# QuanjianSong/UniVST

Measured on AMD Instinct MI355X. Metric: stylized frames/sec, SD-v1.5 16x512x512 @50 DDIM steps, higher is better.
Workload: dtype f16; 1 GPU; sd15_unet_three_branch_pnp_transfer_16x512x512_50ddim; frames=16, branches=3, schedule_steps=53 (wrapping modulo 50), masks=moving disc, blended on steps 0..45, parallelism=single, weights=random-init SD-v1.5 architecture (859M + 201M temporal params), fp16

## Files before the change

### include/univst.h

```cpp
#ifndef UNIVST_H
#define UNIVST_H
#include <stdint.h>
#ifdef __cplusplus
extern "C" {
#endif

#define UNIVST_OK 0
#define UNIVST_ERR_ARG (-1)
#define UNIVST_ERR_HIP (-2)
#define UNIVST_ERR_UNSUPPORTED (-3)
#define UNIVST_ERR_STATE (-4)

#define UNIVST_F16 0
#define UNIVST_F32 1

const char* univst_last_error(void);
#define UNIVST_ABI_VERSION 3
int univst_abi_version(void);

typedef struct univst_unet univst_unet;

typedef struct {
    int in_channels, out_channels;
    int block_out_channels[4];
// ... 146 lines not shown
int univst_motion_load_tensor(univst_motion* h, const char* key, const void* dev_ptr, int dtype, const int64_t* shape, int ndim, void* stream);
int univst_motion_finalize(univst_motion* h, void* stream);
int univst_motion_forward(univst_motion* h, const void* X, void* Y, int B, int F, int N, void* stream);
int univst_motion_query(univst_motion* h, const char* name, double* out);
int univst_temporal_attention(const void* qkv, int64_t ldx, const void* pe_qkv, int B, int F, int N, int heads, int head_dim, void* out, int64_t ldo,
                              void* stream);

int univst_linear(const void* X, int64_t ldx, const void* W, const void* bias, const void* residual, int64_t ldr,
                  void* Y, int64_t ldy, int M, int N, int K, int geglu, void* stream);
int univst_geglu_xres_permute(const void* in, void* out, int rows, int cols, void* stream);
int univst_linear_gated(const void* X, int64_t ldx, const void* W, const void* bias, const void* residual, int64_t ldr, void* Y, int64_t ldy,
                        int M, int N, int K, int act, const void* gate, int64_t ld_gate, int rows_per_gate, void* stream);
int univst_linear_ln(const void* X, int64_t ldx, const void* W, const void* bias, const void* residual, int64_t ldr,
                     void* Y, int64_t ldy, int M, int N, int K, int geglu, const float* ln_stats, float ln_eps,
                     const float* ln_wsum, const float* ln_bias, float* stats_out, void* stream);
int64_t univst_attn2_fused_workspace_bytes(int B, int heads, int head_dim);
int univst_attn2_fused(const void* X, int64_t ldx, const float* ln_stats, float ln_eps, const float* ln_wsum, const float* ln_bias,
                       const void* Wq_frag, int q_prescaled, const void* kv, int B, int T, int64_t rows_per_branch, const void* Wo_frag,
                       const void* bias_o, const void* residual, int64_t ldr, void* Y, int64_t ldy, int64_t M, int C, int heads,
                       float* stats_out, void* workspace, void* stream);
int univst_attn12_fused(const void* attn_out, int64_t ldx, const void* Wp_frag, const void* bias_p, const void* residual_in, int64_t ldr_in, float ln_eps,
                        const float* ln_wsum, const float* ln_bias, const void* Wq_frag, int q_prescaled, const void* kv, int B, int T,
                        int64_t rows_per_branch, const void* Wo_frag, const void* bias_o, void* Y, int64_t ldy, int64_t M, int C, int heads,
                        float* stats_out, void* workspace, void* stream);
int univst_frag_pack(const void* W, void* out, int N, int K, void* stream);
int univst_conv_nhwc(const void* X1, const void* X2, int C1, int C2, int imgs, int Hs, int Ws, int upsample, int stride,
                     int taps, const void* W, const void* bias, const void* rowbias, int rows_per_rowbias,
                     const void* residual, void* Y, int Cout, void* stream);
int univst_conv_nhwc_tapinner(const void* X1, const void* X2, int C1, int C2, int imgs, int Hs, int Ws, int upsample, int stride,
                              const void* W, const void* bias, const void* rowbias, int rows_per_rowbias,
// ... 89 lines not shown
#define UNIVST_PLAN_LN_STATS 8
#define UNIVST_PLAN_STATS_OUT 16
#define UNIVST_PLAN_ACT 32
#define UNIVST_PLAN_GATE 64
#define UNIVST_PLAN_W32_ONLY 128
#define UNIVST_PLAN_W32 256
#define UNIVST_PLAN_GN_OUT 512
#define UNIVST_PLAN_TAPINNER 1024
#define UNIVST_PLAN_Y_UNALIGNED 2048
#define UNIVST_PLAN_WORKSPACE 4096
#define UNIVST_PLAN_GEOM_3X3 0
#define UNIVST_PLAN_GEOM_PAD_END 1
#define UNIVST_PLAN_GEOM_FRAME 2
int univst_debug_gemm_plan(int ncu, int mode, int M, int N, int K, int geglu, int flags, int rows_per_set, int C1, int C2, int Hs, int Ws, int upsample,
                           int stride, int taps, int geom, char* buf, int n);
#define UNIVST_PLAN_SRC_LOGW 1
#define UNIVST_PLAN_EXTRA_KEYS 2
int univst_debug_attention_plan(int BF, int heads, int Nq, int Nkv, int nsrc, int d, int q_prescaled, int flags, int phase, char* buf, int n);

#define UNIVST_GN_PLAN_INTS 16
int univst_debug_groupnorm_plan(int C1, int C2, int64_t rows, int rows_per_stat, int G, int has_fold, int world, int has_producer_stats, int* out_ints);

#ifdef __cplusplus
}
#endif
#endif
```

### univst_amd/_native.py

```python
import ctypes as C
import os
from typing import Optional

import torch

_LIB_PATH = os.environ.get("UNIVST_LIB") or os.path.join(os.path.dirname(os.path.abspath(__file__)), "lib", "libunivst_hip.so")
_lib = None


class UnetCfg(C.Structure):
    _fields_ = [("in_channels", C.c_int), ("out_channels", C.c_int), ("block_out_channels", C.c_int * 4),
                ("layers_per_block", C.c_int), ("cross_attention_dim", C.c_int), ("attention_heads", C.c_int * 4),
                ("norm_num_groups", C.c_int), ("norm_eps", C.c_float), ("flip_sin_to_cos", C.c_int),
                ("freq_shift", C.c_float)]


class ClipCfg(C.Structure):
    _fields_ = [("vocab_size", C.c_int), ("hidden_size", C.c_int), ("intermediate_size", C.c_int), ("num_layers", C.c_int), ("num_heads", C.c_int),
                ("max_positions", C.c_int), ("hidden_act", C.c_int), ("layer_norm_eps", C.c_float), ("projection_dim", C.c_int), ("eos_token_id", C.c_int)]


class T5Cfg(C.Structure):
    _fields_ = [("vocab_size", C.c_int), ("d_model", C.c_int), ("d_ff", C.c_int), ("num_layers", C.c_int), ("num_heads", C.c_int), ("d_kv", C.c_int),
                ("num_buckets", C.c_int), ("max_distance", C.c_int), ("layer_norm_eps", C.c_float)]
# ... 49 lines not shown
    "univst_unet_set_option": (_I, [_P, C.c_char_p, _I]),
    "univst_unet_query": (_I, [_P, C.c_char_p, C.POINTER(C.c_double)]),
    "univst_comm_create": (_I, [_I, _I, _L, C.POINTER(_P)]),
    "univst_comm_handle_bytes": (_I, []),
    "univst_comm_export": (_I, [_P, _P]),
    "univst_comm_connect": (_I, [_P, _P]),
    "univst_comm_connect_local": (_I, [_P, C.POINTER(_P)]),
    "univst_comm_connect_emulated": (_I, [_P, C.c_double, C.c_double]),
    "univst_comm_query": (_I, [_P, C.c_char_p, C.POINTER(C.c_double)]),
    "univst_comm_destroy": (_I, [_P]),
    "univst_comm_allreduce_f32": (_I, [_P, _P, _I, _P]),
    "univst_comm_status": (_I, [_P]),
    "univst_unet_set_comm_native": (_I, [_P, _P]),
    "univst_linear": (_I, [_P, _L, _P, _P, _P, _L, _P, _L, _I, _I, _I, _I, _P]),
    "univst_linear_ln": (_I, [_P, _L, _P, _P, _P, _L, _P, _L, _I, _I, _I, _I, _P, _F, _P, _P, _P, _P]),
    "univst_geglu_xres_permute": (_I, [_P, _P, _I, _I, _P]),
    "univst_frag_pack": (_I, [_P, _P, _I, _I, _P]),
    "univst_vae_create": (_I, [_P, C.POINTER(_P)]),
    "univst_vae_destroy": (_I, [_P]),
    "univst_vae_load_tensor": (_I, [_P, C.c_char_p, _P, _I, C.POINTER(C.c_int64), _I, _P]),
    "univst_vae_finalize": (_I, [_P, _P]),
    "univst_vae_decode": (_I, [_P, _P, _L, _I, _I, _I, _P, _P]),
    "univst_vae_encode": (_I, [_P, _P, _L, _I, _I, _P, _P]),
    "univst_klvae_create": (_I, [_P, C.POINTER(_P)]),
    "univst_klvae_destroy": (_I, [_P]),
    "univst_klvae_load_tensor": (_I, [_P, C.c_char_p, _P, _I, C.POINTER(C.c_int64), _I, _P]),
    "univst_klvae_finalize": (_I, [_P, _P]),
    "univst_klvae_decode": (_I, [_P, _P, _L, _I, _I, _P, _P]),
    "univst_klvae_encode": (_I, [_P, _P, _L, _I, _I, _P, _P]),
    "univst_klvae_query": (_I, [_P, C.c_char_p, C.POINTER(C.c_double)]),
# ... 60 lines not shown
    "univst_latent_adain_apply": (_I, [_P, _P, _P, _L, _P, _I, _I, _I, _P]),
    "univst_axpby": (_I, [_P, _P, _P, _F, _F, _L, _P]),
    "univst_mask_blend": (_I, [_P, _P, _P, _P, _I, _L, _P]),
    "univst_mask_resize": (_I, [_P, _P, _I, _I, _I, _I, _I, _P]),
    "univst_maskprop_workspace_bytes": (_L, [_I, _I, _I]),
    "univst_maskprop_frame": (_I, [_P, _P, _P, _P, _I, _I, _I, _I, _F, _I, _P, _P]),
    "univst_maskprop_finalize": (_I, [_P, _P, _I, _I, _I, _I, _I, _P, _P]),
    "univst_warp_accumulate": (_I, [_P, _P, _P, _P, _P, _I, _I, _F, _P]),
    "univst_warp_window_key": (_I, [_P, _P, _I, _I, _I, _I, _I, _I, _F, _P]),
    "univst_latent_window_smooth": (_I, [_P, _P, _I, _I, _I, _I, _I, _F, _P]),
    "univst_accumulate_u8": (_I, [_P, _P, _L, _P]),
    "univst_window_store": (_I, [_P, _F, _P, _L, _P]),
    "univst_debug_tr16": (_I, [_P, _P]),
    "univst_debug_delay_us": (_I, [C.c_double, _P]),
    "univst_debug_gemm_plan": (_I, [_I] * 16 + [C.c_char_p, _I]),
    "univst_debug_attention_plan": (_I, [_I] * 9 + [C.c_char_p, _I]),
    "univst_debug_groupnorm_plan": (_I, [_I, _I, _L, _I, _I, _I, _I, _I, _P]),
    "univst_profile_enable": (_I, [_I]),
    "univst_profile_symbols": (_I, [_I, C.c_char_p, _I]),
    "univst_profile_collect": (_I, [C.POINTER(C.c_double), C.POINTER(_L), C.POINTER(C.c_double), C.POINTER(C.c_double), _I]),
    "univst_profile_collect_aux": (_I, [C.POINTER(C.c_double), _I]),
}


ABI_VERSION = 3


def lib_path() -> str:
    return _LIB_PATH


def load():
    global _lib
    if _lib is None:
        if not os.path.exists(_LIB_PATH):
            raise RuntimeError(f"{_LIB_PATH} not found: build it with `python __graft_entry__.py build` (or `make`); "
                               "univst_amd has no CPU or eager-PyTorch fallback")
        lib = C.CDLL(_LIB_PATH)
        for name, (res, args) in SIGNATURES.items():
            fn = getattr(lib, name)
            fn.restype = res
            fn.argtypes = args
        if lib.univst_abi_version() != ABI_VERSION:
            raise RuntimeError(f"{_LIB_PATH} has ABI version {lib.univst_abi_version()}, this binding was written against {ABI_VERSION} "
                               "(include/univst.h UNIVST_ABI_VERSION): rebuild the library (`make`)")
        _lib = lib
    return _lib


def check(rc: int, what: str = ""):
    if rc != 0:
        msg = load().univst_last_error().decode(errors="replace")
        raise RuntimeError(f"libunivst_hip {what} failed (code {rc}): {msg}")


# ... 102 lines not shown


def linear_ln(x, w, bias=None, residual=None, geglu=False, out=None, ln=None, stats_out=None, eps=1e-5):
    _f16(x), _f16(w)
    M, K = x.shape
    N = w.shape[0]
    No = N // 2 if geglu else N
    if out is None:
        out = torch.empty(M, No, device=x.device, dtype=torch.float16)
    st, ws, lb = ln if ln is not None else (None, None, None)
    for t in (st, ws, lb, stats_out):
        assert t is None or (t.dtype == torch.float32 and t.is_contiguous())
    check(load().univst_linear_ln(ptr(x), K, ptr(w), ptr(bias), ptr(residual), No, ptr(out), No, M, N, K, int(geglu), ptr(st), eps,
                                  ptr(ws), ptr(lb), ptr(stats_out), stream_ptr()), "linear_ln")
    return out


def conv_nhwc(x1, w, bias=None, x2=None, upsample=False, stride=1, rowbias=None, rows_per_rowbias=1, residual=None):
    _f16(x1), _f16(w)
    imgs, Hs, Ws, C1 = x1.shape
    C2 = 0 if x2 is None else x2.shape[-1]
    Cout, taps, _ = w.shape
    He, We = (Hs * 2, Ws * 2) if upsample else (Hs, Ws)
    Ho = (He - 1) // stride + 1 if taps == 9 else He
    Wo = (We - 1) // stride + 1 if taps == 9 else We
    out = torch.empty(imgs, Ho, Wo, Cout, device=x1.device, dtype=torch.float16)
    check(load().univst_conv_nhwc(ptr(x1), ptr(x2), C1, C2, imgs, Hs, Ws, int(upsample), stride, taps, ptr(w), ptr(bias),
                                  ptr(rowbias), rows_per_rowbias, ptr(residual), ptr(out), Cout, stream_ptr()), "conv_nhwc")
    return out

# ... 315 lines not shown
```

### univst_amd/csrc/abi.hip

```cpp
#include <math.h>
#include <stdarg.h>
#include <stdlib.h>
#include <string.h>

#include <new>

#include "../../include/univst.h"
#include "comm.h"
#include "kernels.h"
#include "unet.h"
#include "vae.h"
#include "raft.h"
#include "clip.h"
#include "t5.h"
#include "motion.h"

static thread_local char g_err[1024] = "";
void uv_set_error(const char* fmt, ...) {
    va_list ap;
    va_start(ap, fmt);
    vsnprintf(g_err, sizeof(g_err), fmt, ap);
    va_end(ap);
}
const char* uv_get_error() { return g_err; }
// ... 42 lines not shown
}
int univst_unet_set_option(univst_unet* h, const char* name, int value) {
    UV_REQUIRE(h && name, "unet_set_option: null argument");
    if (!strcmp(name, "ln_fold")) {
        UV_REQUIRE(value >= 0 && value <= 2, "unet_set_option: ln_fold is 0, 1 or 2");
        h->impl.ln_fold = value;
        return UV_OK;
    }
    if (!strcmp(name, "gn_fold")) {
        h->impl.gn_fold = value != 0;
        return UV_OK;
    }
    if (!strcmp(name, "attn2_fused")) {
        UV_REQUIRE(value >= 0 && value <= 2, "unet_set_option: attn2_fused is 0, 1 or 2");
        h->impl.attn2_fused = value;
        return UV_OK;
    }
    if (!strcmp(name, "gn_producer")) {
        h->impl.gn_producer = value != 0;
        return UV_OK;
    }
    if (!strcmp(name, "chain_bands")) {
        UV_REQUIRE(value >= 0 && value <= 64, "unet_set_option: chain_bands is 0 (auto), 1 (off) or a band count <= 64");
        h->impl.chain_bands = value;
        return UV_OK;
    }
    if (!strcmp(name, "kv_overlap")) {
        h->impl.kv_overlap = value != 0;
        return UV_OK;
    }
// ... 440 lines not shown
    return uv_launch_attn2_fused(p, C, S(s));
}
int univst_linear_ln(const void* X, int64_t ldx, const void* W, const void* bias, const void* R, int64_t ldr, void* Y, int64_t ldy,
                     int M, int N, int K, int geglu, const float* ln_stats, float ln_eps, const float* ln_wsum, const float* ln_bias,
                     float* stats_out, void* s) {
    UV_REQUIRE(X && W && Y, "linear_ln: null argument");
    UV_REQUIRE(!ln_stats || (ln_wsum && ln_bias && K % 160 == 0 && !bias), "linear_ln: a folded LayerNorm needs wsum, lnb (which holds the bias) and K %% 160 == 0");
    UV_REQUIRE((!stats_out || uv_linear_fold_producer_ok(M, N, K)) && (!ln_stats || geglu == 2 || uv_linear_fold_consumer_ok(M, N, K, geglu != 0)),
               "linear_ln: M=%d N=%d K=%d is not taken by the direct 256x320 path (N %% 320 == 0 and >= 150 tiles) nor by the 128-wide path without split-K", M, N, K);
    GemmParams g;
    g.X = H(X); g.ldx = ldx; g.W = H(W); g.bias = H(bias); g.R = H(R); g.ldr = ldr; g.Y = HM(Y); g.ldy = ldy;
    g.M = M; g.N = N; g.K = K; g.geglu = geglu;
    g.ln_stats = ln_stats; g.ln_slots = K / 160; g.ln_eps = ln_eps; g.ln_wsum = ln_wsum; g.ln_bias = ln_bias; g.stats_out = stats_out;
    return uv_launch_gemm(g, 0, S(s));
}
int univst_conv_nhwc(const void* X1, const void* X2, int C1, int C2, int imgs, int Hs, int Ws, int up, int stride, int taps,
                     const void* W, const void* bias, const void* rowbias, int rows_per_rb, const void* R, void* Y, int Cout,
                     void* s) {
    UV_REQUIRE(X1 && W && Y, "conv: null argument");
    UV_REQUIRE((X2 != nullptr) == (C2 > 0), "conv: X2/C2 mismatch");
    UV_REQUIRE(stride == 1 || stride == 2, "conv: stride %d", stride);
    GemmParams g;
    g.X = H(X1); g.X2 = H(X2); g.C1 = C1; g.C2 = C2; g.Hs = Hs; g.Ws = Ws; g.up = up ? 1 : 0; g.stride = stride; g.taps = taps;
    const int He = Hs << g.up, We = Ws << g.up;
    g.Ho = taps == 9 ? (He - 1) / stride + 1 : He;
    g.Wo = taps == 9 ? (We - 1) / stride + 1 : We;
    g.M = imgs * g.Ho * g.Wo; g.N = Cout; g.K = taps * (C1 + C2);
    g.W = H(W); g.bias = H(bias); g.rowbias = H(rowbias); g.rows_per_rb = rows_per_rb > 0 ? rows_per_rb : 1;
    g.R = H(R); g.ldr = Cout; g.Y = HM(Y); g.ldy = Cout;
    return uv_launch_gemm(g, 1, S(s));
// ... 149 lines not shown
        g.korder = on(UNIVST_PLAN_TAPINNER) ? 1 : 0;
    }
    g.ldy = No; g.ldr = No;
    if (on(UNIVST_PLAN_BIAS)) g.bias = h;
    if (on(UNIVST_PLAN_RESIDUAL)) g.R = h;
    if (on(UNIVST_PLAN_ROWBIAS)) g.rowbias = h;
    if (on(UNIVST_PLAN_LN_STATS)) { g.ln_stats = arena; g.ln_wsum = arena; g.ln_bias = arena; g.ln_slots = g.K / 160; }
    if (on(UNIVST_PLAN_STATS_OUT)) g.stats_out = arena;
    if (on(UNIVST_PLAN_ACT)) g.act = 1;
    if (on(UNIVST_PLAN_GATE)) { g.gate = h; g.ld_gate = N; }
    if (on(UNIVST_PLAN_GN_OUT)) { g.gn_out = arena; g.gn_gw = 10; g.gn_G = N / 10; }
    if (on(UNIVST_PLAN_WORKSPACE)) { g.partial = arena; g.partial_bytes = UV_SPLITK_WS_BYTES; }
    if (rows_per_set > 0) { g.w_rows_per_set = rows_per_set; g.bias32 = arena; }
    return uv_gemm_plan_text(g, mode, ncu, buf, n);
}
int univst_debug_attention_plan(int BF, int heads, int Nq, int Nkv, int nsrc, int d, int q_prescaled, int flags, int phase, char* buf, int n) {
    UV_REQUIRE(buf && n > 0 && phase >= 0 && phase <= 2, "debug_attention_plan: null buffer or phase outside 0..2");
    if (Nq == 0 && Nkv == 0) {
        snprintf(buf, (size_t)n, "%s", uv_attention_plan_symbols().c_str());
        return UV_OK;
    }
    alignas(16) static float arena[8];
    half_t* const h = (half_t*)arena;
    AttnParams a;
    a.q = a.k = a.v = h; a.o = h; a.ldq = a.ldkv = a.ldo = (long)heads * d; a.src_idx = (const int*)arena;
    a.nsrc = nsrc; a.BF = BF; a.Nq = Nq; a.Nkv = Nkv; a.heads = heads; a.d = d; a.q_prescaled = q_prescaled != 0;
    if (flags & UNIVST_PLAN_SRC_LOGW) a.src_logw = arena;
    if (flags & UNIVST_PLAN_EXTRA_KEYS) { a.kx = a.vx = h; a.x_idx = (const int*)arena; a.ldkv_x = a.ldkv; a.Nkv_x = 77; }
    if (phase == 1) a.state_out = arena;
    if (phase == 2) a.state_in = arena;
// ... 72 lines not shown
```

### univst_amd/csrc/kernels.h

```cpp
#pragma once
#include "common.h"
#include <string>

struct GemmParams {
    const half_t* X = nullptr;
    const half_t* X2 = nullptr;
    const half_t* W = nullptr;
    const half_t* W32 = nullptr;
    half_t* Y = nullptr;
    long ldx = 0, ldy = 0;
    int M = 0, N = 0, K = 0;
    int C1 = 0, C2 = 0, Hs = 1, Ws = 1, up = 0, Ho = 1, Wo = 1, stride = 1, taps = 1;
    int tapw = 0, pady = 0, padx = 0;
    int korder = 0;
    const half_t* bias = nullptr;
    const half_t* rowbias = nullptr;
    int rows_per_rb = 1;
    long ldrb = 0;
    const half_t* R = nullptr;
    long ldr = 0;
    const half_t* bias2 = nullptr;
    int geglu = 0;
    int act = 0;
    const half_t* gate = nullptr;
// ... 93 lines not shown
struct AttnPlan : UvLaunchPlan {};
GemmPlan uv_gemm_plan(const GemmParams& p, int mode, int ncu);
AttnPlan uv_attention_plan(const AttnParams& p);
int uv_gemm_plan_text(const GemmParams& p, int mode, int ncu, char* buf, int n);
int uv_attention_plan_text(const AttnParams& p, char* buf, int n);
std::string uv_gemm_plan_symbols();
std::string uv_attention_plan_symbols();

int uv_num_cus();
int uv_launch_gemm(const GemmParams& p, int mode, hipStream_t stream);
bool uv_linear_takes_big_direct(long M, int N, int K, long ldx = 0);
bool uv_linear_fold_producer_ok(long M, int N, int K);
bool uv_linear_fold_consumer_ok(long M, int N, int K, bool geglu);
bool uv_geglu_xres_ok(int N, int K, long M = 0);
int uv_launch_geglu_xres_permute(const half_t* in, half_t* out, int rows, int cols, hipStream_t stream);
constexpr size_t UV_SPLITK_WS_BYTES = 128u << 20;
int uv_launch_linear_small(const half_t* x, const half_t* W, const half_t* b, half_t* y, int M, int N, int K, int silu_in,
                           hipStream_t stream);
struct UvGnComm {
    int world = 1;
    float* red = nullptr;
    long byte_off = 0;
    int (*allreduce)(void* user, int64_t byte_off, int count_f32) = nullptr;
    void* user = nullptr;
};
int uv_groupnorm_workspace_floats(int S, int G);
struct UvGnFold {
    const half_t* W = nullptr;
    const half_t* bias = nullptr;
    int N = 0;
// ... 77 lines not shown
```

### univst_amd/csrc/unet.h

```cpp
#pragma once
#include <string>
#include <unordered_map>

#include "../../include/univst.h"
#include "model.h"

struct UNet : WeightStore {
    univst_unet_cfg cfg;
    std::unordered_map<long, int*> idx_tables;
    std::unordered_map<std::string, long> temb_off;
    long temb_total = 0;
    Arena arena;
    bool finalized = false;
    int gn_producer = 1;
    int chain_bands = 1;
    int gn_fold = 1;
    int attn2_fused = 2;
    int ln_fold = 2;
    unsigned* d_counter = nullptr;
    std::unordered_map<std::string, int> temporal_conv_active;
    std::unordered_map<std::string, int> temporal_attn_active;
    int rank = 0, world = 1;
    univst_allreduce_fn allreduce = nullptr;
    univst_kv_exchange_fn kv_exchange = nullptr;
    void* comm_user = nullptr;
    char* comm_ws = nullptr;
    long comm_ws_bytes = 0;
    struct univst_comm* native_comm = nullptr;
    int kv_overlap = 1;
    int emu_wire_gbps = 0, emu_wire_lat_us = 3;
    double emu_wire_us = 0.0;
    hipStream_t xstream = nullptr;
// ... 14 lines not shown
```

### univst_amd/csrc/unet.hip

```cpp
#include <math.h>
#include <string.h>

#include <map>
#include <string>
#include <unordered_map>
#include <vector>

#include "comm.h"
#include "kernels.h"
#include "unet.h"

namespace {

__global__ void permute_conv_weight_t32_kernel(const half_t* __restrict__ in, half_t* __restrict__ out, int Co, int Ci) {
    long i = (long)blockIdx.x * blockDim.x + threadIdx.x;
    long total = (long)Co * Ci * 9;
    if (i >= total) return;
    int j = (int)(i % 32);
    int t = (int)((i / 32) % 9);
    int q = (int)((i / (32 * 9)) % (Ci / 32));
    int o = (int)(i / ((long)Ci * 9));
    out[i] = in[((long)o * Ci + q * 32 + j) * 9 + t];
}
__global__ void geglu_interleave_kernel(const half_t* __restrict__ in, half_t* __restrict__ out, int rows, int cols) {
// ... 618 lines not shown
        g.R = R;
        g.ldr = ldr;
        g.bias2 = bias2;
        g.geglu = geglu;
        if (!g.W || (!bkey.empty() && !ln_in && !wsets && !g.bias)) return u.missing_error("unet");
        g.partial = sk_ws;
        g.partial_bytes = UV_SPLITK_WS_BYTES;
        UV_RUN(uv_launch_gemm(g, 0, s));
        if (g.gn_out) {
            if (emitted) *gst_out = g.gn_out;
            else gst_give_back(M, N);
        }
        return UV_OK;
    }

    struct KvSlots {
        long o_send = 0, o_first = 0, o_prev = 0, o_rfirst = 0, nbytes = 0;
        bool emu = false;
    } kvs;
    int kv_post(const half_t* h, int C, int N) {
        kvs = KvSlots();
        kvs.nbytes = (long)B * N * C * sizeof(half_t);
        const int nslot = u.native_comm ? 6 : 4;
        const long slot = ((u.comm_ws_bytes - 65536) / nslot) & ~255L;
        UV_REQUIRE(kvs.nbytes <= slot, "kv_exchange: comm workspace too small (%ld B per slot, need %ld)", slot, kvs.nbytes);
        const long par = u.native_comm ? uv_comm_kv_parity(u.native_comm) : 0;
        kvs.o_send = 65536;
        kvs.o_first = kvs.o_send + slot;
        kvs.o_prev = kvs.o_first + slot * (1 + 2 * par);
        kvs.o_rfirst = kvs.o_prev + slot;
// ... 100 lines not shown
        if (gnf) {
            free(wsets);
            free(b32);
        }
        half_t *gm, *bt;
        gm = W(b + ".norm1.weight"); bt = W(b + ".norm1.bias");
        if (!gm || !bt) return u.missing_error("unet");
        if (!fold) UV_RUN(uv_launch_layernorm(h, C, t0, C, gm, bt, rows, C, 1e-5f, s));
        const bool shard = u.world > 1, halo = shard && u.rank > 0;
        if (shard) UV_RUN(kv_post(h, C, N));
        const long extra_rows = shard ? (long)2 * B * N : 0;
        half_t* qkv = alloc((rows + extra_rows) * 3 * C);
        if (!qkv) return UV_ERR_STATE;
        const bool qs = u.find(b + ".attn1.qkv#fused#qs") != nullptr;
        const std::string wqkv = b + (qs ? ".attn1.qkv#fused#qs" : ".attn1.qkv#fused");
        if (fold) UV_RUN(linear(h, C, rows, C, wqkv + "#ln", "", 3 * C, qkv, 3 * C, nullptr, 0, nullptr, 0, nullptr, lnst));
        else UV_RUN(linear(t0, C, rows, C, wqkv, "", 3 * C, qkv, 3 * C));
        const bool registered = pnp_layer && pnp && pnp->registered;
        const bool shift = registered && pnp->idx >= pnp->eta1 && pnp->idx <= pnp->eta2 * 50.f;
        float beta = 0.f;
        if (shift) {
            UV_REQUIRE(B == 3, "PnP attention shift needs the three-branch batch (B=3), got B=%d", B);
            beta = (0.9f - 0.1f) / (pnp->eta1 * 50.f - pnp->eta2 * 50.f) * ((float)pnp->idx - pnp->eta2 * 50.f) + 0.1f;
            UV_RUN(uv_launch_adain_shift(qkv, 3 * C, F, N, C, ad_ws, ad_ws + (long)F * 2 * C, pnp->alpha, beta, pnp->gamma, s));
        }
        AttnParams ap;
        ap.q = qkv; ap.k = qkv + C; ap.v = qkv + 2 * C;
        ap.ldq = ap.ldkv = 3 * C;
        ap.o = t0; ap.ldo = C;
        ap.src_idx = registered ? idx_pnp : idx_stock;
        ap.src_cnt = registered ? cnt_pnp : cnt_stock;
        ap.src_logw = registered ? lw_pnp : lw_stock;
// ... 119 lines not shown
            else UV_RUN(linear(t0 + o, C, brows, C, wq2, "", C, q2, C));
            ap.q = q2; ap.ldq = C;
            ap.k = kv; ap.v = kv + C; ap.ldkv = 2 * C;
            ap.o = t0 + o; ap.ldo = C;
            ap.src_idx = idx_text + bd * band_imgs; ap.src_cnt = nullptr; ap.src_logw = nullptr; ap.nsrc = 1; ap.Nkv = text_len;
            ap.BF = band_imgs;
            ap.q_prescaled = qs2;
            UV_RUN(uv_launch_attention(ap, s));
            if (nbands == 1) { free(q2); free(kv); }
            if (!h3 && !(h3 = alloc(rows * C))) return UV_ERR_STATE;
            UV_RUN(linear(t0 + o, C, brows, C, b + ".attn2.to_out.0.weight", b + ".attn2.to_out.0.bias", C, h3 + o, C, h2 + o, C, nullptr, 0, fold3 ? lb : nullptr));
            if (nbands == 1) free(h2);
            }
            }
            if (!mid && !(mid = alloc(brows * 4 * C))) return UV_ERR_STATE;
            const bool xres = u.find(b + ".ff.net.0.proj.weight#xres") != nullptr && uv_geglu_xres_ok(8 * C, C, brows);
            const std::string wff = b + (xres ? ".ff.net.0.proj.weight#xres" : ".ff.net.0.proj.weight#geglu");
            const std::string bff = b + (xres ? ".ff.net.0.proj.bias#xres" : ".ff.net.0.proj.bias#geglu");
            if (!fold3) {
                UV_RUN(uv_launch_layernorm(h3 + o, C, t0 + o, C, gm3, bt3, brows, C, 1e-5f, s));
                UV_RUN(linear(t0 + o, C, brows, C, wff, bff, 8 * C, mid, 4 * C, nullptr, 0, nullptr, xres ? 2 : 1));
            } else {
                UV_RUN(linear(h3 + o, C, brows, C, wff + "#ln", "", 8 * C, mid, 4 * C, nullptr, 0, nullptr, xres ? 2 : 1, nullptr, lb));
            }
            if (nbands == 1 && lnst) free(lnst);
            if (!h4 && !(h4 = alloc(rows * C))) return UV_ERR_STATE;
            UV_RUN(linear(mid, 4 * C, brows, 4 * C, b + ".ff.net.2.weight", b + ".ff.net.2.bias", C, h4 + o, C, h3 + o, C, t_attn ? nullptr : tb));
        }
        ap.BF = x.imgs;
        if (nbands > 1) {
            free(h);
            free(q2);
            free(kv);
            free(h2);
            if (lnst) free(lnst);
        }
        free(mid);
        free(h3);
// ... 187 lines not shown
```

Before: 5.857 frames/s.

## Add weight-stationary K=320 linear kernel for large-M transformer projections

Adds a new GEMM kernel specialised for K=320 in which each block keeps a 320-column weight slice in registers and streams many 64-row tiles of activations through LDS, with a triple-buffered global-to-LDS pipeline. It supports an optional folded LayerNorm and bias epilogue. Dispatch uses a 'wins' predicate that routes the fused QKV projection to it when M is large, and the kernel is on by default. GEGLU is excluded from the 'wins' predicate, so the FF projection stays on the old path by default. The aim is to avoid re-reading weights per tile and to cut overhead for the 320-channel layers, at the cost of high register pressure at one block per CU.

After: 5.915 frames/s (median of 6 runs). About the same (+1.0%).

```diff
diff --git a/include/univst.h b/include/univst.h
--- a/include/univst.h
+++ b/include/univst.h
@@ -184,6 +184,8 @@
 int univst_linear_ln(const void* X, int64_t ldx, const void* W, const void* bias, const void* residual, int64_t ldr,
                      void* Y, int64_t ldy, int M, int N, int K, int geglu, const float* ln_stats, float ln_eps,
                      const float* ln_wsum, const float* ln_bias, float* stats_out, void* stream);
+int univst_linear_ws(const void* X, int64_t ldx, const void* W, const void* bias, void* Y, int64_t ldy, int M, int N, int K, int geglu,
+                     const float* ln_stats, float ln_eps, const float* ln_wsum, const float* ln_bias, void* stream);
 int64_t univst_attn2_fused_workspace_bytes(int B, int heads, int head_dim);
 int univst_attn2_fused(const void* X, int64_t ldx, const float* ln_stats, float ln_eps, const float* ln_wsum, const float* ln_bias,
                        const void* Wq_frag, int q_prescaled, const void* kv, int B, int T, int64_t rows_per_branch, const void* Wo_frag,
@@ -303,6 +305,18 @@
 #define UNIVST_PLAN_GEOM_FRAME 2
 int univst_debug_gemm_plan(int ncu, int mode, int M, int N, int K, int geglu, int flags, int rows_per_set, int C1, int C2, int Hs, int Ws, int upsample,
                            int stride, int taps, int geom, char* buf, int n);
+#define UNIVST_LWS_BIAS 1
+#define UNIVST_LWS_GEGLU_XRES 2
+#define UNIVST_LWS_LN_FOLD 4
+#define UNIVST_LWS_RESIDUAL 8
+#define UNIVST_LWS_BIAS2 16
+#define UNIVST_LWS_STATS_OUT 32
+#define UNIVST_LWS_GN_OUT 64
+#define UNIVST_LWS_WEIGHT_SETS 128
+#define UNIVST_LWS_GEGLU_BLOCKS 256
+#define UNIVST_LWS_ROWS_UNALIGNED 512
+#define UNIVST_LWS_PREDICATE_ONLY 1024
+int univst_debug_linear_ws_plan(int ncu, int M, int N, int K, int flags, char* buf, int n);
 #define UNIVST_PLAN_SRC_LOGW 1
 #define UNIVST_PLAN_EXTRA_KEYS 2
 int univst_debug_attention_plan(int BF, int heads, int Nq, int Nkv, int nsrc, int d, int q_prescaled, int flags, int phase, char* buf, int n);
diff --git a/univst_amd/_native.py b/univst_amd/_native.py
--- a/univst_amd/_native.py
+++ b/univst_amd/_native.py
@@ -87,6 +87,7 @@
     "univst_unet_set_comm_native": (_I, [_P, _P]),
     "univst_linear": (_I, [_P, _L, _P, _P, _P, _L, _P, _L, _I, _I, _I, _I, _P]),
     "univst_linear_ln": (_I, [_P, _L, _P, _P, _P, _L, _P, _L, _I, _I, _I, _I, _P, _F, _P, _P, _P, _P]),
+    "univst_linear_ws": (_I, [_P, _L, _P, _P, _P, _L, _I, _I, _I, _I, _P, _F, _P, _P, _P]),
     "univst_geglu_xres_permute": (_I, [_P, _P, _I, _I, _P]),
     "univst_frag_pack": (_I, [_P, _P, _I, _I, _P]),
     "univst_vae_create": (_I, [_P, C.POINTER(_P)]),
@@ -177,6 +178,7 @@
     "univst_debug_tr16": (_I, [_P, _P]),
     "univst_debug_delay_us": (_I, [C.c_double, _P]),
     "univst_debug_gemm_plan": (_I, [_I] * 16 + [C.c_char_p, _I]),
+    "univst_debug_linear_ws_plan": (_I, [_I] * 5 + [C.c_char_p, _I]),
     "univst_debug_attention_plan": (_I, [_I] * 9 + [C.c_char_p, _I]),
     "univst_debug_groupnorm_plan": (_I, [_I, _I, _L, _I, _I, _I, _I, _I, _P]),
     "univst_profile_enable": (_I, [_I]),
@@ -187,6 +189,7 @@
 
 
 ABI_VERSION = 3
+ADDED_SINCE_ABI_3 = {"univst_linear_ws", "univst_debug_linear_ws_plan"}
 
 
 def lib_path() -> str:
@@ -201,7 +204,11 @@
                                "univst_amd has no CPU or eager-PyTorch fallback")
         lib = C.CDLL(_LIB_PATH)
         for name, (res, args) in SIGNATURES.items():
-            fn = getattr(lib, name)
+            fn = getattr(lib, name, None)
+            if fn is None:
+                if name in ADDED_SINCE_ABI_3:
+                    continue
+                raise RuntimeError(f"{_LIB_PATH} does not export {name} (include/univst.h): rebuild the library (`make`)")
             fn.restype = res
             fn.argtypes = args
         if lib.univst_abi_version() != ABI_VERSION:
@@ -334,6 +341,38 @@
     check(load().univst_linear_ln(ptr(x), K, ptr(w), ptr(bias), ptr(residual), No, ptr(out), No, M, N, K, int(geglu), ptr(st), eps,
                                   ptr(ws), ptr(lb), ptr(stats_out), stream_ptr()), "linear_ln")
     return out
+
+
+def linear_ws(x, w, bias=None, geglu=False, out=None, ln=None, M=None, eps=1e-5):
+    _f16(w)
+    for name, t in (("x", x), ("out", out)):
+        if t is not None and not (t.is_cuda and t.dtype == torch.float16 and t.dim() == 2 and t.stride(1) == 1):
+            raise ValueError(f"linear_ws: {name} must be fp16 CUDA/HIP rows with contiguous columns, got {t.dtype} {t.device} strides {t.stride()}")
+    M = x.shape[0] if M is None else M
+    N, K = w.shape
+    No = N // 2 if geglu else N
+    if out is None:
+        out = torch.empty(M, No, device=x.device, dtype=torch.float16)
+    if x.shape[0] < M or out.shape[0] < M or x.shape[1] < K or out.shape[1] < No:
+        raise ValueError(f"linear_ws: M={M} rows of {K} -> {No} columns do not fit x {tuple(x.shape)} / out {tuple(out.shape)}")
+    st, ws, lb = ln if ln is not None else (None, None, None)
+    for t in (st, ws, lb):
+        assert t is None or (t.dtype == torch.float32 and t.is_contiguous())
+    check(load().univst_linear_ws(ptr(x), x.stride(0), ptr(w), ptr(bias), ptr(out), out.stride(0), M, N, K, int(geglu), ptr(st), eps, ptr(ws), ptr(lb),
+                                  stream_ptr()), "linear_ws")
+    return out
+
+
+def linear_ws_plan(ncu, M, N, K, flags=0):
+    buf = C.create_string_buffer(512)
+    rc = load().univst_debug_linear_ws_plan(ncu, M, N, K, flags, buf, 512)
+    if rc != 0:
+        raise RuntimeError(buf.value.decode())
+    return buf.value.decode()
+
+
+LWS_BIAS, LWS_GEGLU_XRES, LWS_LN_FOLD, LWS_RESIDUAL, LWS_BIAS2, LWS_STATS_OUT, LWS_GN_OUT, LWS_WEIGHT_SETS, LWS_GEGLU_BLOCKS, LWS_ROWS_UNALIGNED, LWS_PREDICATE_ONLY = (
+    1, 2, 4, 8, 16, 32, 64, 128, 256, 512, 1024)
 
 
 def conv_nhwc(x1, w, bias=None, x2=None, upsample=False, stride=1, rowbias=None, rows_per_rowbias=1, residual=None):
diff --git a/univst_amd/csrc/abi.hip b/univst_amd/csrc/abi.hip
--- a/univst_amd/csrc/abi.hip
+++ b/univst_amd/csrc/abi.hip
@@ -80,6 +80,11 @@
     if (!strcmp(name, "attn2_fused")) {
         UV_REQUIRE(value >= 0 && value <= 2, "unet_set_option: attn2_fused is 0, 1 or 2");
         h->impl.attn2_fused = value;
+        return UV_OK;
+    }
+    if (!strcmp(name, "linear_ws")) {
+        UV_REQUIRE(value >= 0 && value <= 2, "unet_set_option: linear_ws is 0, 1 or 2");
+        h->impl.linear_ws = value;
         return UV_OK;
     }
     if (!strcmp(name, "gn_producer")) {
@@ -550,6 +555,15 @@
     g.ln_stats = ln_stats; g.ln_slots = K / 160; g.ln_eps = ln_eps; g.ln_wsum = ln_wsum; g.ln_bias = ln_bias; g.stats_out = stats_out;
     return uv_launch_gemm(g, 0, S(s));
 }
+int univst_linear_ws(const void* X, int64_t ldx, const void* W, const void* bias, void* Y, int64_t ldy, int M, int N, int K, int geglu,
+                     const float* ln_stats, float ln_eps, const float* ln_wsum, const float* ln_bias, void* s) {
+    UV_REQUIRE(X && W && Y, "linear_ws: null argument");
+    GemmParams g;
+    g.X = H(X); g.ldx = ldx; g.W = H(W); g.bias = H(bias); g.Y = HM(Y); g.ldy = ldy;
+    g.M = M; g.N = N; g.K = K; g.geglu = geglu;
+    g.ln_stats = ln_stats; g.ln_slots = ln_stats ? K / 160 : 0; g.ln_eps = ln_eps; g.ln_wsum = ln_wsum; g.ln_bias = ln_bias;
+    return uv_launch_linear_ws(g, S(s));
+}
 int univst_conv_nhwc(const void* X1, const void* X2, int C1, int C2, int imgs, int Hs, int Ws, int up, int stride, int taps,
                      const void* W, const void* bias, const void* rowbias, int rows_per_rb, const void* R, void* Y, int Cout,
                      void* s) {
@@ -729,6 +743,35 @@
     if (rows_per_set > 0) { g.w_rows_per_set = rows_per_set; g.bias32 = arena; }
     return uv_gemm_plan_text(g, mode, ncu, buf, n);
 }
+int univst_debug_linear_ws_plan(int ncu, int M, int N, int K, int flags, char* buf, int n) {
+    UV_REQUIRE(buf && n > 0 && ncu > 0, "debug_linear_ws_plan: null buffer or ncu <= 0");
+    if (M == 0 && N == 0) {
+        snprintf(buf, (size_t)n, "%s", uv_linear_ws_plan_symbols().c_str());
+        return UV_OK;
+    }
+    if (flags & UNIVST_LWS_PREDICATE_ONLY) {
+        const int f = flags & ~UNIVST_LWS_PREDICATE_ONLY;
+        snprintf(buf, (size_t)n, "ok=%d wins=%d", (int)uv_linear_ws_ok(M, N, K, f), (int)uv_linear_ws_wins(M, N, K, f));
+        return UV_OK;
+    }
+    alignas(16) static float arena[8];
+    half_t* const h = (half_t*)arena;
+    auto on = [&](int bit) { return (flags & bit) != 0; };
+    GemmParams g;
+    g.X = g.W = h; g.Y = h;
+    g.M = M; g.N = N; g.K = K;
+    g.geglu = on(UNIVST_LWS_GEGLU_XRES) ? 2 : (on(UNIVST_LWS_GEGLU_BLOCKS) ? 1 : 0);
+    g.ldx = on(UNIVST_LWS_ROWS_UNALIGNED) ? K + 4 : K;
+    g.ldy = g.geglu ? N / 2 : N;
+    if (on(UNIVST_LWS_BIAS)) g.bias = h;
+    if (on(UNIVST_LWS_LN_FOLD)) { g.ln_stats = arena; g.ln_wsum = arena; g.ln_bias = arena; g.ln_slots = K / 160; g.ln_eps = 1e-5f; }
+    if (on(UNIVST_LWS_RESIDUAL)) { g.R = h; g.ldr = g.ldy; }
+    if (on(UNIVST_LWS_BIAS2)) g.bias2 = h;
+    if (on(UNIVST_LWS_STATS_OUT)) g.stats_out = arena;
+    if (on(UNIVST_LWS_GN_OUT)) { g.gn_out = arena; g.gn_gw = 10; g.gn_G = N / 10; }
+    if (on(UNIVST_LWS_WEIGHT_SETS)) { g.w_rows_per_set = 256; g.bias32 = arena; }
+    return uv_linear_ws_plan_text(g, ncu, buf, n);
+}
 int univst_debug_attention_plan(int BF, int heads, int Nq, int Nkv, int nsrc, int d, int q_prescaled, int flags, int phase, char* buf, int n) {
     UV_REQUIRE(buf && n > 0 && phase >= 0 && phase <= 2, "debug_attention_plan: null buffer or phase outside 0..2");
     if (Nq == 0 && Nkv == 0) {
diff --git a/univst_amd/csrc/kernels.h b/univst_amd/csrc/kernels.h
--- a/univst_amd/csrc/kernels.h
+++ b/univst_amd/csrc/kernels.h
@@ -131,6 +131,16 @@
 bool uv_linear_fold_consumer_ok(long M, int N, int K, bool geglu);
 bool uv_geglu_xres_ok(int N, int K, long M = 0);
 int uv_launch_geglu_xres_permute(const half_t* in, half_t* out, int rows, int cols, hipStream_t stream);
+enum { UV_LWS_BIAS = 1, UV_LWS_GEGLU_XRES = 2, UV_LWS_LN_FOLD = 4, UV_LWS_RESIDUAL = 8, UV_LWS_BIAS2 = 16, UV_LWS_STATS_OUT = 32, UV_LWS_GN_OUT = 64, UV_LWS_WEIGHT_SETS = 128 };
+struct LinearWsPlan : UvLaunchPlan {
+    int slices = 0, chunks = 0, spc = 0, nstages = 0;
+};
+LinearWsPlan uv_linear_ws_plan(const GemmParams& p, int ncu);
+bool uv_linear_ws_ok(long M, int N, int K, int flags);
+bool uv_linear_ws_wins(long M, int N, int K, int flags);
+int uv_launch_linear_ws(const GemmParams& p, hipStream_t stream);
+int uv_linear_ws_plan_text(const GemmParams& p, int ncu, char* buf, int n);
+std::string uv_linear_ws_plan_symbols();
 constexpr size_t UV_SPLITK_WS_BYTES = 128u << 20;
 int uv_launch_linear_small(const half_t* x, const half_t* W, const half_t* b, half_t* y, int M, int N, int K, int silu_in,
                            hipStream_t stream);
diff --git a/univst_amd/csrc/linear_ws.hip b/univst_amd/csrc/linear_ws.hip
--- /dev/null
+++ b/univst_amd/csrc/linear_ws.hip
@@ -0,0 +1,334 @@
+#include <string.h>
+#include <type_traits>
+
+#include "common.h"
+#include "kernels.h"
+
+namespace {
+
+__device__ __attribute__((aligned(256))) half_t lws_zero_page[128];
+
+struct LwsArgs {
+    const half_t* X;
+    const half_t* W;
+    const half_t* bias;
+    half_t* Y;
+    const float* ln_stats;
+    const float* ln_wsum;
+    const float* ln_bias;
+    long ldx, ldy;
+    int M, slices, nstages, spc;
+    float ln_eps;
+};
+
+constexpr int LWS_K = 320, LWS_BM = 64, LWS_NKT = LWS_K / 64;
+constexpr int LWS_STAGE = LWS_NKT * LWS_BM * 64;
+constexpr int LWS_SLD = 88;
+constexpr int LWS_SLAB = 16 * LWS_SLD;
+
+template <int EPI, int LNF>
+__global__ __launch_bounds__(256, 1) void linear_ws_kernel(LwsArgs p) {
+    __shared__ __attribute__((aligned(16))) half_t smem[3 * LWS_STAGE + 4 * 2 * LWS_SLAB + (LNF == 2 ? 4 * 3 * 512 + 4 * 320 : 0)];
+    const int tid = threadIdx.x, lane = tid & 63, wave = tid >> 6;
+    const int l15 = lane & 15, g = lane >> 4;
+    const int wave_u = __builtin_amdgcn_readfirstlane(wave);
+    half_t* const slab0 = smem + 3 * LWS_STAGE + wave_u * 2 * LWS_SLAB;
+    half_t* const lnslot = smem + 3 * LWS_STAGE + 4 * 2 * LWS_SLAB + wave_u * 3 * 512;
+    const int lid = xcd_remap(blockIdx.x, gridDim.x);
+    const int slice = lid % p.slices, chunk = lid / p.slices;
+    const int s_begin = chunk * p.spc;
+    const int nst = min(p.spc, p.nstages - s_begin);
+    if (nst <= 0) return;
+    auto glds16 = [&](const half_t* src, half_t* dst) {
+        __builtin_amdgcn_global_load_lds((const __attribute__((address_space(1))) void*)src, (__attribute__((address_space(3))) void*)dst, 16, 0, 0);
+    };
+    const int rb = tid >> 3, kc = (tid & 7) ^ (rb & 7);
+    auto issue = [&](int st, int buf) {
+#pragma unroll
+        for (int i = 0; i < 2; ++i) {
+            const long m = (long)st * LWS_BM + rb + 32 * i;
+            const half_t* src = p.X + m * p.ldx + kc * 8;
+            const bool ok = m < p.M;
+#pragma unroll
+            for (int kt = 0; kt < LWS_NKT; ++kt)
+                glds16(ok ? src + kt * 64 : lws_zero_page, smem + buf * LWS_STAGE + kt * LWS_BM * 64 + (32 * i + wave_u * 8) * 64);
+        }
+        if constexpr (LNF == 2) {
+            const long m = (long)st * LWS_BM + lane;
+            glds16(m < p.M ? reinterpret_cast<const half_t*>(p.ln_stats + m * 4) : lws_zero_page, lnslot + buf * 512);
+        }
+    };
+    issue(s_begin, 0);
+    if (nst > 1) issue(s_begin + 1, 1);
+
+    const int n0 = slice * 320 + wave * 80;
+    h8 w[5][10];
+#pragma unroll
+    for (int i = 0; i < 5; ++i)
+#pragma unroll
+        for (int ks = 0; ks < 10; ++ks) w[i][ks] = *reinterpret_cast<const h8*>(p.W + (long)(n0 + i * 16 + l15) * LWS_K + ks * 32 + g * 8);
+    f4 cb[LNF == 2 ? 1 : 5];
+    float* const cst = reinterpret_cast<float*>(smem + 3 * LWS_STAGE + 4 * 2 * LWS_SLAB + 4 * 3 * 512) + wave_u * 160;
+    if constexpr (LNF == 2) {
+        for (int c = lane; c < 160; c += 64) cst[c] = c < 80 ? p.ln_wsum[n0 + c] : p.ln_bias[n0 + c - 80];
+        __builtin_amdgcn_fence(__ATOMIC_RELEASE, "wavefront");
+        __builtin_amdgcn_wave_barrier();
+        __builtin_amdgcn_fence(__ATOMIC_ACQUIRE, "wavefront");
+    } else {
+#pragma unroll
+        for (int i = 0; i < 5; ++i) {
+            h4 b = {0, 0, 0, 0};
+            if (p.bias) b = *reinterpret_cast<const h4*>(p.bias + n0 + i * 16 + g * 4);
+            cb[i] = f4{(float)b[0], (float)b[1], (float)b[2], (float)b[3]};
+        }
+    }
+
+    const int sw = l15 & 7;
+    auto load_b = [&](const half_t* Xs, int j, h8 (&b)[10]) {
+#pragma unroll
+        for (int ks = 0; ks < 10; ++ks)
+            b[ks] = *reinterpret_cast<const h8*>(&Xs[(ks >> 1) * LWS_BM * 64 + (j * 16 + l15) * 64 + ((((ks & 1) * 4 + g) ^ sw) * 8)]);
+    };
+    auto finish = [&](const f4 (&acc)[5], long m0, float2 ln, half_t* slab, bool full) {
+        if constexpr (EPI == 0) {
+#pragma unroll
+            for (int i = 0; i < 5; ++i) {
+                f4 v = acc[i];
+                if constexpr (LNF == 2) {
+                    const f4 cw = *reinterpret_cast<const f4*>(cst + i * 16 + g * 4), cl = *reinterpret_cast<const f4*>(cst + 80 + i * 16 + g * 4);
+#pragma unroll
+                    for (int r = 0; r < 4; ++r) v[r] = fmaf(ln.y, fmaf(-ln.x, cw[r], v[r]), cl[r]);
+                } else {
+                    v += cb[i];
+                }
+                *reinterpret_cast<h4*>(&slab[l15 * LWS_SLD + i * 16 + g * 4]) = h4{(half_t)v[0], (half_t)v[1], (half_t)v[2], (half_t)v[3]};
+            }
+        } else {
+#pragma unroll
+            for (int i = 0; i < 5; ++i) {
+                f4 v = acc[i];
+                if constexpr (LNF == 2) {
+                    const f4 cw = *reinterpret_cast<const f4*>(cst + i * 16 + g * 4), cl = *reinterpret_cast<const f4*>(cst + 80 + i * 16 + g * 4);
+#pragma unroll
+                    for (int r = 0; r < 4; ++r) v[r] = fmaf(ln.y, fmaf(-ln.x, cw[r], v[r]), cl[r]);
+                } else {
+                    v += cb[i];
+                }
+                const f2 y = geglu_erf2(f2{v[0], v[1]}, f2{v[2], v[3]});
+                *reinterpret_cast<h2*>(&slab[l15 * LWS_SLD + i * 8 + g * 2]) = h2{(half_t)y.x, (half_t)y.y};
+            }
+        }
+        __builtin_amdgcn_fence(__ATOMIC_RELEASE, "wavefront");
+        __builtin_amdgcn_wave_barrier();
+        __builtin_amdgcn_fence(__ATOMIC_ACQUIRE, "wavefront");
+        constexpr int CPR = EPI == 0 ? 10 : 5;
+        constexpr int NCH = 16 * CPR, NFULL = NCH / 64, NTAIL = NCH % 64;
+        half_t* const yb = p.Y + (EPI == 0 ? n0 : n0 / 2);
+#pragma unroll
+        for (int it = 0; it < NFULL; ++it) {
+            const int id = it * 64 + lane;
+            const int row = id / CPR, c = id - row * CPR;
+            const h8 v = *reinterpret_cast<const h8*>(&slab[row * LWS_SLD + c * 8]);
+            if (full || m0 + row < p.M) *reinterpret_cast<h8*>(yb + (m0 + row) * p.ldy + c * 8) = v;
+        }
+        constexpr int PPC = 64 / NTAIL, PH = 8 / PPC;
+        const int id = NFULL * 64 + lane / PPC, row = id / CPR, col = (id - row * CPR) * 8 + (lane % PPC) * PH;
+        if constexpr (PH == 4) {
+            const h4 v = *reinterpret_cast<const h4*>(&slab[row * LWS_SLD + col]);
+            if (full || m0 + row < p.M) *reinterpret_cast<h4*>(yb + (m0 + row) * p.ldy + col) = v;
+        } else {
+            const h2 v = *reinterpret_cast<const h2*>(&slab[row * LWS_SLD + col]);
+            if (full || m0 + row < p.M) *reinterpret_cast<h2*>(yb + (m0 + row) * p.ldy + col) = v;
+        }
+    };
+
+    f4 pend[5];
+#pragma unroll
+    for (int i = 0; i < 5; ++i) pend[i] = f4{0.f, 0.f, 0.f, 0.f};
+    long pend_m0 = p.M;
+    float2 pend_ln = float2{0.f, 1.f};
+    float2 lnc = float2{0.f, 1.f};
+    auto stage = [&](auto full_c, const half_t* Xs, long ms) {
+        constexpr bool FULL = decltype(full_c)::value;
+        h8 b[10];
+        load_b(Xs, 0, b);
+#pragma unroll
+        for (int j = 0; j < 4; ++j) {
+            f4 acc[5];
+#pragma unroll
+            for (int i = 0; i < 5; ++i) acc[i] = f4{0.f, 0.f, 0.f, 0.f};
+#pragma unroll
+            for (int ks = 0; ks < 10; ++ks)
+#pragma unroll
+                for (int i = 0; i < 5; ++i) acc[i] = __builtin_amdgcn_mfma_f32_16x16x32_f16(w[i][ks], b[ks], acc[i], 0, 0, 0);
+            float2 ln = float2{0.f, 1.f};
+            if constexpr (LNF == 2) {
+                ln.x = __shfl(lnc.x, j * 16 + l15, 64);
+                ln.y = __shfl(lnc.y, j * 16 + l15, 64);
+            }
+            if (j < 3) load_b(Xs, j + 1, b);
+            finish(pend, pend_m0, pend_ln, slab0 + (j & 1) * LWS_SLAB, FULL);
+#pragma unroll
+            for (int k = 0; k < 10; ++k) {
+                __builtin_amdgcn_sched_group_barrier(0x008, 1, 0);
+                __builtin_amdgcn_sched_group_barrier(0x100, 1, 0);
+            }
+#pragma unroll
+            for (int k = 0; k < 40; ++k) {
+                __builtin_amdgcn_sched_group_barrier(0x008, 1, 0);
+                __builtin_amdgcn_sched_group_barrier(0x002, EPI == 0 ? 3 : 6, 0);
+            }
+#pragma unroll
+            for (int i = 0; i < 5; ++i) pend[i] = acc[i];
+            pend_m0 = ms + j * 16;
+            pend_ln = ln;
+        }
+    };
+    constexpr int GL = LNF == 2 ? 11 : 10;
+    constexpr int ST4 = 4 * (EPI == 0 ? 3 : 2);
+    auto wait_vm = [&](int n) {
+#define UV_VMCNT(N) __builtin_amdgcn_s_waitcnt(((N) & 15) | (7 << 4) | (15 << 8) | (((N) >> 4) << 14))
+        switch (n) {
+            case GL: UV_VMCNT(GL); break;
+            case ST4: UV_VMCNT(ST4); break;
+            case GL + ST4: UV_VMCNT(GL + ST4); break;
+            case 2 * ST4: UV_VMCNT(2 * ST4); break;
+            case GL + 2 * ST4: UV_VMCNT(GL + 2 * ST4); break;
+            default: UV_VMCNT(0); break;
+        }
+#undef UV_VMCNT
+    };
+    bool full_1 = false, full_2 = false;
+    for (int it = 0; it < nst; ++it) {
+        wait_vm(it == 0 ? 0 : (full_2 ? ST4 : 0) + (it + 1 < nst ? GL : 0) + (full_1 ? ST4 : 0));
+        __builtin_amdgcn_s_barrier();
+        if (it + 2 < nst) issue(s_begin + it + 2, (it + 2) % 3);
+        if constexpr (LNF == 2) {
+            const f4 lnraw = *reinterpret_cast<const f4*>(lnslot + (it % 3) * 512 + lane * 8);
+            const float mean = (lnraw[0] + lnraw[2]) * (1.f / LWS_K);
+            const float var = fmaxf(fmaf(-mean, mean, (lnraw[1] + lnraw[3]) * (1.f / LWS_K)), 0.f);
+            lnc = float2{mean, rsqrtf(var + p.ln_eps)};
+        }
+        const half_t* Xs = smem + (it % 3) * LWS_STAGE;
+        const long ms = (long)(s_begin + it) * LWS_BM;
+        const bool full = it > 0 && ms + LWS_BM <= p.M;
+        if (full) stage(std::true_type{}, Xs, ms);
+        else stage(std::false_type{}, Xs, ms);
+        full_2 = full_1;
+        full_1 = full;
+    }
+    finish(pend, pend_m0, pend_ln, slab0, false);
+}
+
+struct LwsKernel {
+    void (*fn)(LwsArgs);
+    const char* sym;
+};
+#define UV_KERNEL(...) {__VA_ARGS__, #__VA_ARGS__}
+const LwsKernel LWS_KERNELS[] = {
+    UV_KERNEL(linear_ws_kernel<0,0>), UV_KERNEL(linear_ws_kernel<0,2>), UV_KERNEL(linear_ws_kernel<1,0>), UV_KERNEL(linear_ws_kernel<1,2>),
+};
+#undef UV_KERNEL
+
+}
+
+LinearWsPlan uv_linear_ws_plan(const GemmParams& p, int ncu) {
+    LinearWsPlan pl;
+    auto al16 = [](const void* q) { return (reinterpret_cast<uintptr_t>(q) & 15) == 0; };
+    UV_PLAN_REQUIRE(pl, p.M > 0 && p.N > 0 && ncu > 0, "linear_ws: empty problem M=%d N=%d K=%d", p.M, p.N, p.K);
+    UV_PLAN_REQUIRE(pl, p.K == LWS_K, "linear_ws: K=%d, the weight-stationary kernel holds K = 320 in registers", p.K);
+    UV_PLAN_REQUIRE(pl, p.N % 320 == 0, "linear_ws: N=%d must be a multiple of 320 (four waves of 80 columns)", p.N);
+    UV_PLAN_REQUIRE(pl, p.geglu == 0 || p.geglu == 2, "linear_ws: GEGLU needs the weights in the X-resident row order (geglu = 2), got geglu = %d", p.geglu);
+    UV_PLAN_REQUIRE(pl, !p.R && !p.rowbias, "linear_ws: no residual / row bias epilogue (M=%d N=%d)", p.M, p.N);
+    UV_PLAN_REQUIRE(pl, !p.bias2, "linear_ws: no second bias epilogue (M=%d N=%d)", p.M, p.N);
+    UV_PLAN_REQUIRE(pl, !p.stats_out, "linear_ws: no row-statistics output (M=%d N=%d)", p.M, p.N);
+    UV_PLAN_REQUIRE(pl, !p.gn_out, "linear_ws: no GroupNorm-statistics output (M=%d N=%d)", p.M, p.N);
+    UV_PLAN_REQUIRE(pl, !p.w_rows_per_set && !p.bias32, "linear_ws: no weight sets / fp32 bias (M=%d N=%d)", p.M, p.N);
+    UV_PLAN_REQUIRE(pl, !p.act && !p.gate, "linear_ws: no activation / gate epilogue (M=%d N=%d)", p.M, p.N);
+    UV_PLAN_REQUIRE(pl, !p.ln_stats || (p.ln_wsum && p.ln_bias && p.ln_slots == 2 && !p.bias),
+                    "linear_ws: a folded LayerNorm needs ln_wsum, ln_bias (which carries the bias) and the 2 statistics slots of K = 320, got %d", p.ln_slots);
+    UV_PLAN_REQUIRE(pl, p.X && p.W && p.Y, "linear_ws: null operand");
+    UV_PLAN_REQUIRE(pl, p.ldx >= LWS_K && p.ldx % 8 == 0 && p.ldy % 8 == 0 && p.ldy >= (p.geglu ? p.N / 2 : p.N) && al16(p.X) && al16(p.W) && al16(p.Y) &&
+                    (reinterpret_cast<uintptr_t>(p.bias) & 7) == 0 && al16(p.ln_stats) && al16(p.ln_wsum) && al16(p.ln_bias),
+                    "linear_ws: rows must be 16-byte aligned (ldx=%ld ldy=%ld multiples of 8, ldx >= 320, ldy >= the output width)", p.ldx, p.ldy);
+    pl.slices = p.N / 320;
+    pl.nstages = (p.M + LWS_BM - 1) / LWS_BM;
+    int best_chunks = 1;
+    double best = 1e30;
+    for (int R = 1; R <= 8; ++R) {
+        int chunks = (int)((long)R * ncu / pl.slices);
+        if (chunks < 1) chunks = 1;
+        if (chunks > pl.nstages) chunks = pl.nstages;
+        int spc = (pl.nstages + chunks - 1) / chunks;
+        if (spc < 8 && R > 1) break;
+        if (spc < 8) spc = pl.nstages < 8 ? pl.nstages : 8;
+        chunks = (pl.nstages + spc - 1) / spc;
+        const long blocks = (long)chunks * pl.slices;
+        const double cost = (double)((blocks + ncu - 1) / ncu) * (spc + 2);
+        if (cost < best) { best = cost; best_chunks = chunks; }
+        if (chunks == pl.nstages) break;
+    }
+    pl.spc = (pl.nstages + best_chunks - 1) / best_chunks;
+    pl.chunks = (pl.nstages + pl.spc - 1) / pl.spc;
+    pl.grid = (unsigned)(pl.chunks * pl.slices);
+    pl.block = 256;
+    pl.cls = UV_CLS_GEMM_BIG;
+    pl.flops = 2.0 * p.M * (double)p.N * p.K;
+    pl.bytes = 2.0 * ((double)p.M * p.K + (double)p.N * p.K + (double)p.M * (p.geglu ? p.N / 2 : p.N));
+    snprintf(pl.sym, sizeof pl.sym, "linear_ws_kernel<%d,%d>", p.geglu ? 1 : 0, p.ln_stats ? 2 : 0);
+    return pl;
+}
+
+bool uv_linear_ws_ok(long M, int N, int K, int flags) {
+    return M > 0 && M < (1L << 31) && N > 0 && K == LWS_K && N % 320 == 0 && (flags & ~(UV_LWS_BIAS | UV_LWS_GEGLU_XRES | UV_LWS_LN_FOLD)) == 0 &&
+           !((flags & UV_LWS_BIAS) && (flags & UV_LWS_LN_FOLD));
+}
+
+bool uv_linear_ws_wins(long M, int N, int K, int flags) {
+    if (!uv_linear_ws_ok(M, N, K, flags) || (flags & UV_LWS_GEGLU_XRES)) return false;
+    return (flags & UV_LWS_LN_FOLD) ? M >= 196608 : M >= 65536;
+}
+
+int uv_launch_linear_ws(const GemmParams& p, hipStream_t stream) {
+    const LinearWsPlan pl = uv_linear_ws_plan(p, uv_num_cus());
+    if (pl.rc != UV_OK) {
+        uv_set_error("%s", pl.err);
+        return pl.rc;
+    }
+    const LwsKernel* kern = nullptr;
+    for (const LwsKernel& k : LWS_KERNELS)
+        if (!strcmp(k.sym, pl.sym)) kern = &k;
+    if (!kern) {
+        uv_set_error("linear_ws: the plan names %s, which the launch table does not hold", pl.sym);
+        return UV_ERR_STATE;
+    }
+    LwsArgs a;
+    a.X = p.X; a.W = p.W; a.bias = p.bias; a.Y = p.Y;
+    a.ln_stats = p.ln_stats; a.ln_wsum = p.ln_wsum; a.ln_bias = p.ln_bias;
+    a.ldx = p.ldx; a.ldy = p.ldy;
+    a.M = p.M; a.slices = pl.slices; a.nstages = pl.nstages; a.spc = pl.spc;
+    a.ln_eps = p.ln_eps;
+    uv_prof_begin(pl.cls, pl.flops, pl.bytes, stream, pl.sym);
+    hipLaunchKernelGGL(kern->fn, dim3(pl.grid), dim3(pl.block), 0, stream, a);
+    uv_prof_end(stream);
+    UV_LAUNCH_CHECK();
+    return UV_OK;
+}
+
+int uv_linear_ws_plan_text(const GemmParams& p, int ncu, char* buf, int n) {
+    const LinearWsPlan pl = uv_linear_ws_plan(p, ncu);
+    if (pl.rc != UV_OK) {
+        snprintf(buf, (size_t)n, "%s", pl.err);
+        uv_set_error("%s", pl.err);
+        return pl.rc;
+    }
+    const int flags = (p.bias ? UV_LWS_BIAS : 0) | (p.geglu ? UV_LWS_GEGLU_XRES : 0) | (p.ln_stats ? UV_LWS_LN_FOLD : 0);
+    snprintf(buf, (size_t)n, "%s grid=%u block=%u slices=%d chunks=%d stages_per_chunk=%d stages=%d ok=%d wins=%d", pl.sym, pl.grid, pl.block, pl.slices, pl.chunks,
+             pl.spc, pl.nstages, (int)uv_linear_ws_ok(p.M, p.N, p.K, flags), (int)uv_linear_ws_wins(p.M, p.N, p.K, flags));
+    return UV_OK;
+}
+std::string uv_linear_ws_plan_symbols() {
+    std::string out;
+    for (const LwsKernel& k : LWS_KERNELS) out += (out.empty() ? "" : ";") + std::string(k.sym);
+    return out;
+}
diff --git a/univst_amd/csrc/unet.h b/univst_amd/csrc/unet.h
--- a/univst_amd/csrc/unet.h
+++ b/univst_amd/csrc/unet.h
@@ -16,6 +16,7 @@
     int chain_bands = 1;
     int gn_fold = 1;
     int attn2_fused = 2;
+    int linear_ws = 1;
     int ln_fold = 2;
     unsigned* d_counter = nullptr;
     std::unordered_map<std::string, int> temporal_conv_active;
diff --git a/univst_amd/csrc/unet.hip b/univst_amd/csrc/unet.hip
--- a/univst_amd/csrc/unet.hip
+++ b/univst_amd/csrc/unet.hip
@@ -656,6 +656,30 @@
         return UV_OK;
     }
 
+    bool ws_takes(long M, int N, int K, int flags) const {
+        return u.linear_ws == 2 ? uv_linear_ws_ok(M, N, K, flags) : (u.linear_ws == 1 && uv_linear_ws_wins(M, N, K, flags));
+    }
+    int linear_k320(const half_t* X, long ldx, long M, int K, const std::string& wkey, const std::string& bkey, int N, half_t* Y, long ldy, int geglu,
+                    const float* ln_in) {
+        const int flags = (!bkey.empty() && !ln_in ? UV_LWS_BIAS : 0) | (geglu == 2 ? UV_LWS_GEGLU_XRES : 0) | (ln_in ? UV_LWS_LN_FOLD : 0);
+        if ((geglu != 0 && geglu != 2) || !ws_takes(M, N, K, flags))
+            return linear(X, ldx, M, K, wkey, bkey, N, Y, ldy, nullptr, 0, nullptr, geglu, nullptr, ln_in);
+        GemmParams g;
+        g.X = X; g.ldx = ldx; g.M = (int)M; g.K = K; g.N = N; g.Y = Y; g.ldy = ldy; g.geglu = geglu;
+        g.W = W(wkey);
+        g.bias = (bkey.empty() || ln_in) ? nullptr : W(bkey);
+        if (ln_in) {
+            g.ln_stats = ln_in;
+            g.ln_slots = K / 160;
+            g.ln_eps = 1e-5f;
+            g.ln_wsum = (const float*)W(wkey + ".wsum");
+            g.ln_bias = (const float*)W(wkey + ".bias");
+            if (!g.ln_wsum || !g.ln_bias) return u.missing_error("unet");
+        }
+        if (!g.W || (!bkey.empty() && !ln_in && !g.bias)) return u.missing_error("unet");
+        return uv_launch_linear_ws(g, s);
+    }
+
     struct KvSlots {
         long o_send = 0, o_first = 0, o_prev = 0, o_rfirst = 0, nbytes = 0;
         bool emu = false;
@@ -786,8 +810,8 @@
         if (!qkv) return UV_ERR_STATE;
         const bool qs = u.find(b + ".attn1.qkv#fused#qs") != nullptr;
         const std::string wqkv = b + (qs ? ".attn1.qkv#fused#qs" : ".attn1.qkv#fused");
-        if (fold) UV_RUN(linear(h, C, rows, C, wqkv + "#ln", "", 3 * C, qkv, 3 * C, nullptr, 0, nullptr, 0, nullptr, lnst));
-        else UV_RUN(linear(t0, C, rows, C, wqkv, "", 3 * C, qkv, 3 * C));
+        if (fold) UV_RUN(linear_k320(h, C, rows, C, wqkv + "#ln", "", 3 * C, qkv, 3 * C, 0, lnst));
+        else UV_RUN(linear_k320(t0, C, rows, C, wqkv, "", 3 * C, qkv, 3 * C, 0, nullptr));
         const bool registered = pnp_layer && pnp && pnp->registered;
         const bool shift = registered && pnp->idx >= pnp->eta1 && pnp->idx <= pnp->eta2 * 50.f;
         float beta = 0.f;
@@ -937,14 +961,15 @@
             }
             }
             if (!mid && !(mid = alloc(brows * 4 * C))) return UV_ERR_STATE;
-            const bool xres = u.find(b + ".ff.net.0.proj.weight#xres") != nullptr && uv_geglu_xres_ok(8 * C, C, brows);
+            const bool xres = u.find(b + ".ff.net.0.proj.weight#xres") != nullptr &&
+                              (uv_geglu_xres_ok(8 * C, C, brows) || ws_takes(brows, 8 * C, C, UV_LWS_GEGLU_XRES | (fold3 ? UV_LWS_LN_FOLD : UV_LWS_BIAS)));
             const std::string wff = b + (xres ? ".ff.net.0.proj.weight#xres" : ".ff.net.0.proj.weight#geglu");
             const std::string bff = b + (xres ? ".ff.net.0.proj.bias#xres" : ".ff.net.0.proj.bias#geglu");
             if (!fold3) {
                 UV_RUN(uv_launch_layernorm(h3 + o, C, t0 + o, C, gm3, bt3, brows, C, 1e-5f, s));
-                UV_RUN(linear(t0 + o, C, brows, C, wff, bff, 8 * C, mid, 4 * C, nullptr, 0, nullptr, xres ? 2 : 1));
+                UV_RUN(linear_k320(t0 + o, C, brows, C, wff, bff, 8 * C, mid, 4 * C, xres ? 2 : 1, nullptr));
             } else {
-                UV_RUN(linear(h3 + o, C, brows, C, wff + "#ln", "", 8 * C, mid, 4 * C, nullptr, 0, nullptr, xres ? 2 : 1, nullptr, lb));
+                UV_RUN(linear_k320(h3 + o, C, brows, C, wff + "#ln", "", 8 * C, mid, 4 * C, xres ? 2 : 1, lb));
             }
             if (nbands == 1 && lnst) free(lnst);
             if (!h4 && !(h4 = alloc(rows * C))) return UV_ERR_STATE;
```
